# huiscliu/lssp

Hardware: AMD Instinct MI355X
Metric: fp64 CSR SpMV GB/s (% HBM peak) + BiCGSTAB iters/s, 7-pt Poisson n=10M (higher is better)
Workload: dtype f64; 1 GPU; 7-pt Poisson 216^3 (n=10077696, nnz=70263936), BiCGSTAB + ILUK(0), b=1, x0=0, fp64 CSR int32; rows=10077696, partition=1 z-slab row blocks, reduction=tree, transport=none, comm_ranks=1

## Files before the change

### include/lssp_amd.h

```cpp
#ifndef LSSP_AMD_H
#define LSSP_AMD_H

#ifdef __cplusplus
extern "C" {
#endif

enum {
    LSSP_AMD_OK = 0,
    LSSP_AMD_EINVAL = 1,
    LSSP_AMD_EHIP = 2,
    LSSP_AMD_ENOMEM = 3,
    LSSP_AMD_ETIMEOUT = 4,
    LSSP_AMD_ECOMM = 5,
    LSSP_AMD_EUNSUPPORTED = 6
};

enum {
    LSSP_AMD_REDUCE_SERIAL = 0,
    LSSP_AMD_REDUCE_TREE = 1
};

enum {
    LSSP_AMD_GMRES = 0, LSSP_AMD_LGMRES = 1, LSSP_AMD_RGMRES = 2, LSSP_AMD_RLGMRES = 3, LSSP_AMD_BICGSTAB = 4,
    LSSP_AMD_BICGSAFE = 6, LSSP_AMD_CG = 7, LSSP_AMD_CGS = 8, LSSP_AMD_GPBICG = 9, LSSP_AMD_CR = 10,
// ... 9 lines not shown

const char *lssp_amd_strerror(int status);
int lssp_amd_version(void);

void lssp_amd_set_print(int (*fn)(void *user, const char *msg), void *user);

int lssp_amd_ctx_create(int device, lssp_amd_ctx **ctx);
int lssp_amd_ctx_destroy(lssp_amd_ctx *ctx);
int lssp_amd_ctx_set_reduction(lssp_amd_ctx *ctx, int mode);
int lssp_amd_ctx_sync(lssp_amd_ctx *ctx);
void *lssp_amd_ctx_stream(lssp_amd_ctx *ctx);

int lssp_amd_vec_alloc(lssp_amd_ctx *ctx, long n, double **d);
int lssp_amd_vec_free(lssp_amd_ctx *ctx, double *d);
int lssp_amd_vec_upload(lssp_amd_ctx *ctx, double *d, const double *h, long n);
int lssp_amd_vec_download(lssp_amd_ctx *ctx, double *h, const double *d, long n);

int lssp_amd_csr_sort_columns(int nrows, int ncols, int *Ap, int *Aj, double *Ax);
int lssp_amd_mat_upload(lssp_amd_ctx *ctx, int nrows, int ncols, int nnz, const int *Ap,
                        const int *Aj, const double *Ax, lssp_amd_mat **A);
int lssp_amd_mat_destroy(lssp_amd_mat *A);
int lssp_amd_mat_info(const lssp_amd_mat *A, int *nrows, int *ncols, int *nnz);
int lssp_amd_mat_layout(const lssp_amd_mat *A, int *ndiag, int *windowed);
int lssp_amd_mat_bytes(const lssp_amd_mat *A, long long *csr_bytes, long long *aux_bytes);

int lssp_amd_mv_amxpby(lssp_amd_ctx *ctx, double alpha, const lssp_amd_mat *A, double *x,
                       double beta, double *y);
int lssp_amd_mv_amxpbyz(lssp_amd_ctx *ctx, double alpha, const lssp_amd_mat *A, double *x,
                        double beta, const double *y, double *z);
int lssp_amd_mv_amxy(lssp_amd_ctx *ctx, double a, const lssp_amd_mat *A, double *x, double *y);
int lssp_amd_mv_mxy(lssp_amd_ctx *ctx, const lssp_amd_mat *A, double *x, double *y);

int lssp_amd_vec_set_value(lssp_amd_ctx *ctx, double *x, long n, double val);
int lssp_amd_vec_copy(lssp_amd_ctx *ctx, double *x, const double *y, long n);
int lssp_amd_stream_read(lssp_amd_ctx *ctx, const double *x, long n, double *sink);
int lssp_amd_vec_axy(lssp_amd_ctx *ctx, double alpha, const double *x, double *y, long n);
int lssp_amd_vec_axpby(lssp_amd_ctx *ctx, double alpha, const double *x, double beta, double *y,
                       long n);
int lssp_amd_vec_axpbyz(lssp_amd_ctx *ctx, double alpha, const double *x, double beta,
                        const double *y, double *z, long n);
int lssp_amd_vec_scale(lssp_amd_ctx *ctx, double *x, long n, double a);
int lssp_amd_vec_dot(lssp_amd_ctx *ctx, const double *x, const double *y, long n, double *result);
int lssp_amd_vec_norm(lssp_amd_ctx *ctx, const double *x, long n, double *result);

int lssp_amd_ilu_create(lssp_amd_ctx *ctx, int kind, int n, const int *Ap, const int *Aj,
                        const double *Ax, int level, double tol, int p, int blk,
// ... 104 lines not shown
```

### lssp_amd/_lib.py

```python
from __future__ import annotations

import ctypes
import os

HERE = os.path.dirname(os.path.abspath(__file__))
LIB_PATH = os.environ.get("LSSP_AMD_LIB") or os.path.join(HERE, "lib", "liblssp_amd.so")
HEADER = os.path.join(os.path.dirname(HERE), "include", "lssp_amd.h")

_vp, _ci, _cd, _cl = ctypes.c_void_p, ctypes.c_int, ctypes.c_double, ctypes.c_long
_pvp = ctypes.POINTER(ctypes.c_void_p)


ALLGATHER_FN = ctypes.CFUNCTYPE(_ci, _vp, _vp, _vp, _cl)
SENDRECV_FN = ctypes.CFUNCTYPE(_ci, _vp, _ci, ctypes.POINTER(_ci), ctypes.POINTER(_vp), ctypes.POINTER(_cl),
                               _ci, ctypes.POINTER(_ci), ctypes.POINTER(_vp), ctypes.POINTER(_cl))


class HostTransport(ctypes.Structure):
    _fields_ = [("user", _vp), ("allgather", ALLGATHER_FN), ("sendrecv", SENDRECV_FN)]


class SolveParams(ctypes.Structure):
    _fields_ = [("solver", _ci), ("tol_rel", _cd), ("tol_abs", _cd), ("tol_rb", _cd),
                ("maxit", _ci), ("restart", _ci), ("verb", _ci), ("aug_k", _ci),
                ("bgsl", _ci), ("idrs", _ci)]


SIGNATURES = {
    "lssp_amd_strerror": (ctypes.c_char_p, [_ci]),
    "lssp_amd_version": (_ci, []),
    "lssp_amd_set_print": (None, [_vp, _vp]),
    "lssp_amd_ctx_create": (_ci, [_ci, _pvp]),
    "lssp_amd_ctx_destroy": (_ci, [_vp]),
    "lssp_amd_ctx_set_reduction": (_ci, [_vp, _ci]),
    "lssp_amd_ctx_sync": (_ci, [_vp]),
    "lssp_amd_ctx_stream": (_vp, [_vp]),
    "lssp_amd_vec_alloc": (_ci, [_vp, _cl, _pvp]),
    "lssp_amd_vec_free": (_ci, [_vp, _vp]),
    "lssp_amd_vec_upload": (_ci, [_vp, _vp, _vp, _cl]),
    "lssp_amd_vec_download": (_ci, [_vp, _vp, _vp, _cl]),
    "lssp_amd_csr_sort_columns": (_ci, [_ci, _ci, _vp, _vp, _vp]),
    "lssp_amd_mat_upload": (_ci, [_vp, _ci, _ci, _ci, _vp, _vp, _vp, _pvp]),
    "lssp_amd_mat_destroy": (_ci, [_vp]),
    "lssp_amd_mat_info": (_ci, [_vp, _vp, _vp, _vp]),
    "lssp_amd_mat_layout": (_ci, [_vp, _vp, _vp]),
    "lssp_amd_mat_bytes": (_ci, [_vp, _vp, _vp]),
    "lssp_amd_ilu_sweep_layout": (_ci, [_vp, _vp, _vp, _vp]),
    "lssp_amd_mv_amxpby": (_ci, [_vp, _cd, _vp, _vp, _cd, _vp]),
    "lssp_amd_mv_amxpbyz": (_ci, [_vp, _cd, _vp, _vp, _cd, _vp, _vp]),
    "lssp_amd_mv_amxy": (_ci, [_vp, _cd, _vp, _vp, _vp]),
    "lssp_amd_mv_mxy": (_ci, [_vp, _vp, _vp, _vp]),
    "lssp_amd_vec_set_value": (_ci, [_vp, _vp, _cl, _cd]),
    "lssp_amd_vec_copy": (_ci, [_vp, _vp, _vp, _cl]),
    "lssp_amd_stream_read": (_ci, [_vp, _vp, _cl, _vp]),
    "lssp_amd_vec_axy": (_ci, [_vp, _cd, _vp, _vp, _cl]),
    "lssp_amd_vec_axpby": (_ci, [_vp, _cd, _vp, _cd, _vp, _cl]),
    "lssp_amd_vec_axpbyz": (_ci, [_vp, _cd, _vp, _cd, _vp, _vp, _cl]),
    "lssp_amd_vec_scale": (_ci, [_vp, _vp, _cl, _cd]),
    "lssp_amd_vec_dot": (_ci, [_vp, _vp, _vp, _cl, _vp]),
    "lssp_amd_vec_norm": (_ci, [_vp, _vp, _cl, _vp]),
    "lssp_amd_ilu_create": (_ci, [_vp, _ci, _ci, _vp, _vp, _vp, _ci, _cd, _ci, _ci, _pvp]),
    "lssp_amd_ilu_from_factors": (_ci, [_vp, _ci, _vp, _vp, _vp, _vp, _vp, _vp, _pvp]),
    "lssp_amd_bilu_create": (_ci, [_vp, _ci, _vp, _vp, _vp, _ci, _ci, _pvp]),
    "lssp_amd_ilu_from_ldu": (_ci, [_vp, _ci, _vp, _vp, _vp, _vp, _vp, _vp, _vp, _vp, _vp, _pvp]),
    "lssp_amd_ilu_get_diag": (_ci, [_vp, _vp, _vp]),
    "lssp_amd_bilu_factor_host": (_ci, [_ci, _vp, _vp, _vp, _ci, _ci, _vp, _vp, _vp, _vp, _vp, _vp, _vp, _vp, _vp]),
    "lssp_amd_ilu_destroy": (_ci, [_vp]),
    "lssp_amd_ilu_apply": (_ci, [_vp, _vp, _vp, _vp]),
# ... 60 lines not shown
```

### lssp_amd/csrc/capi.cpp

```cpp
#include <hip/hip_runtime.h>

#include <algorithm>
#include <chrono>
#include <climits>
#include <cstdarg>
#include <atomic>
#include <cstdlib>
#include <cstring>
#include <exception>
#include <mutex>
#include <thread>

#include "bilu_dev.h"
#include "internal.h"

using namespace lssp_amd;

namespace lssp_amd {

long num_chunks(long n) { return (n + CHUNK - 1) / CHUNK; }

int ensure_part(lssp_amd_ctx *c, long C)
{
    if (C <= c->part_cap) return LSSP_AMD_OK;
// ... 406 lines not shown

static int check_csr(int nrows, int ncols, int nnz, const int *Ap, const int *Aj)
{
    if (nrows < 0 || ncols <= 0 || nnz < 0 || !Ap) return LSSP_AMD_EINVAL;
    if (Ap[0] != 0 || Ap[nrows] != nnz) return LSSP_AMD_EINVAL;
    for (int i = 0; i < nrows; i++)
        if (Ap[i + 1] < Ap[i]) return LSSP_AMD_EINVAL;
    for (int k = 0; k < nnz; k++)
        if (Aj[k] < 0 || Aj[k] >= ncols) return LSSP_AMD_EINVAL;
    return LSSP_AMD_OK;
}

static int upload_csr(lssp_amd_mat *M, const int *Ap, const int *Aj, const double *Ax)
{
    LSSP_HIP(hipMalloc(&M->Ap, sizeof(int) * (M->nrows + 1)));
    LSSP_HIP(hipMalloc(&M->Aj, sizeof(int) * (M->nnz + 4)));
    LSSP_HIP(hipMalloc(&M->Ax, sizeof(double) * (M->nnz + 4)));
    LSSP_HIP(hipMemcpy(M->Ap, Ap, sizeof(int) * (M->nrows + 1), hipMemcpyHostToDevice));
    if (M->nnz) {
        LSSP_HIP(hipMemcpy(M->Aj, Aj, sizeof(int) * M->nnz, hipMemcpyHostToDevice));
        LSSP_HIP(hipMemcpy(M->Ax, Ax, sizeof(double) * M->nnz, hipMemcpyHostToDevice));
    }
    LSSP_TRY(build_diag_ids(M, Ap, Aj));
    return build_windows(M, Ap, Aj, Ax);
}

int lssp_amd_mat_upload(lssp_amd_ctx *c, int nrows, int ncols, int nnz, const int *Ap, const int *Aj,
                        const double *Ax, lssp_amd_mat **out)
{
    if (!c || !out) return LSSP_AMD_EINVAL;
    LSSP_TRY(check_csr(nrows, ncols, nnz, Ap, Aj));
    LSSP_HIP(hipSetDevice(c->device));
    lssp_amd_mat *M = new lssp_amd_mat();
    M->ctx = c;
    M->nrows = nrows;
    M->ncols = ncols;
    M->nnz = nnz;
    M->n_global = nrows;
    int st = upload_csr(M, Ap, Aj, Ax);
    if (st != LSSP_AMD_OK) {
        lssp_amd_mat_destroy(M);
        return st;
    }
    if (tune_spmv_streams(c, M) != LSSP_AMD_OK) (void)hipGetLastError();
    *out = M;
    return LSSP_AMD_OK;
}

int lssp_amd_mat_destroy(lssp_amd_mat *M)
{
    if (!M) return LSSP_AMD_OK;
    if (M->ctx) (void)hipStreamSynchronize(M->ctx->stream);
    if (M->Ap) (void)hipFree(M->Ap);
    if (M->Aj) (void)hipFree(M->Aj);
    if (M->Ax) (void)hipFree(M->Ax);
    if (M->Ad) (void)hipFree(M->Ad);
    if (M->d_off) (void)hipFree(M->d_off);
    if (M->d_win) (void)hipFree(M->d_win);
    for (void *p : {(void *)M->s_ax, (void *)M->s_col, (void *)M->s_row, (void *)M->s_meta})
        if (p) (void)hipFree(p);
    if (M->d_send_idx) (void)hipFree(M->d_send_idx);
    if (M->d_send_buf) (void)hipFree(M->d_send_buf);
    delete M;
    return LSSP_AMD_OK;
}

int lssp_amd_mat_info(const lssp_amd_mat *A, int *nrows, int *ncols, int *nnz)
{
    if (!A) return LSSP_AMD_EINVAL;
    if (nrows) *nrows = A->nrows;
    if (ncols) *ncols = A->ncols;
    if (nnz) *nnz = A->nnz;
    return LSSP_AMD_OK;
}

int lssp_amd_mat_bytes(const lssp_amd_mat *A, long long *csr_bytes, long long *aux_bytes)
{
    if (!A) return LSSP_AMD_EINVAL;
    if (csr_bytes) *csr_bytes = 4LL * (A->nrows + 1) + 12LL * A->nnz;
    if (aux_bytes) *aux_bytes = A->aux_bytes;
    return LSSP_AMD_OK;
}

int lssp_amd_mat_layout(const lssp_amd_mat *A, int *ndiag, int *windowed)
{
    if (!A || !ndiag) return LSSP_AMD_EINVAL;
    *ndiag = A->ndiag;
    if (windowed) *windowed = A->d_win != nullptr;
    return LSSP_AMD_OK;
}

int lssp_amd_mat_local_rows(const lssp_amd_mat *A, int *row0, int *nlocal, int *nhalo)
{
    if (!A) return LSSP_AMD_EINVAL;
    if (row0) *row0 = A->row0;
    if (nlocal) *nlocal = A->nrows;
    if (nhalo) *nhalo = A->nhalo;
    return LSSP_AMD_OK;
}

int lssp_amd_mv_amxpby(lssp_amd_ctx *c, double alpha, const lssp_amd_mat *A, double *x,
                       double beta, double *y)
{
    if (!c || !A || !x || !y) return LSSP_AMD_EINVAL;
    return spmv_halo(c, A, EPI_AXPBY, alpha, x, beta, y, y, 0, nullptr, nullptr);
}

int lssp_amd_mv_amxpbyz(lssp_amd_ctx *c, double alpha, const lssp_amd_mat *A, double *x,
                        double beta, const double *y, double *z)
{
    if (!c || !A || !x || !y || !z) return LSSP_AMD_EINVAL;
// ... 755 lines not shown
```

### lssp_amd/csrc/comm.cpp

```cpp
#include <hip/hip_runtime.h>
#include <rccl/rccl.h>

#include <algorithm>
#include <climits>
#include <cstring>
#include <map>

#include "internal.h"

namespace lssp_amd {

#define LSSP_NCCL(call)                                                                            \
    do {                                                                                           \
        ncclResult_t r_ = (call);                                                                  \
        if (r_ != ncclSuccess) {                                                                   \
            fprintf(stderr, "lssp_amd: RCCL error %s at %s:%d\n", ncclGetErrorString(r_), __FILE__, \
                    __LINE__);                                                                     \
            return LSSP_AMD_ECOMM;                                                                 \
        }                                                                                          \
    } while (0)

struct Msg {
    int peer;
    void *dbuf;
// ... 458 lines not shown
    if (nsend)
        LSSP_HIP(hipMemcpyAsync(sendg.data(), d_sendg.p, sizeof(int) * nsend, hipMemcpyDeviceToHost, c->stream));
    LSSP_HIP(hipStreamSynchronize(c->stream));
    st = LSSP_AMD_OK;
    for (int &g : sendg) {
        if (g < row0 || g >= row0 + nlocal) st = LSSP_AMD_EINVAL;
        g -= row0;
    }
    LSSP_TRY(agree_status(c, st));
    auto dev_ok = [](hipError_t e) { return e == hipSuccess; };
    const bool ok =
        dev_ok(hipMalloc(&M->d_send_idx, sizeof(int) * std::max(nsend, 1))) &&
        dev_ok(hipMalloc(&M->d_send_buf, sizeof(double) * std::max(nsend, 1))) &&
        (!nsend || dev_ok(hipMemcpy(M->d_send_idx, sendg.data(), sizeof(int) * nsend, hipMemcpyHostToDevice))) &&
        dev_ok(hipMalloc(&M->Ap, sizeof(int) * (nlocal + 1))) &&
        dev_ok(hipMalloc(&M->Aj, sizeof(int) * ((size_t)nnz + 4))) &&
        dev_ok(hipMalloc(&M->Ax, sizeof(double) * ((size_t)nnz + 4))) &&
        dev_ok(hipMemcpy(M->Ap, Ap, sizeof(int) * (nlocal + 1), hipMemcpyHostToDevice)) &&
        (!nnz || (dev_ok(hipMemcpy(M->Aj, lj.data(), sizeof(int) * (size_t)nnz, hipMemcpyHostToDevice)) &&
                  dev_ok(hipMemcpy(M->Ax, Ax, sizeof(double) * (size_t)nnz, hipMemcpyHostToDevice))));
    if (!ok) (void)hipGetLastError();
    LSSP_TRY(agree_status(c, ok ? LSSP_AMD_OK : LSSP_AMD_ENOMEM));
    LSSP_TRY(agree_status(c, build_diag_ids(M, Ap, lj.data())));
    guard.m = nullptr;
    *out = M;
    return LSSP_AMD_OK;
}

}
```

### lssp_amd/csrc/convert.hip

```cpp
#include <hip/hip_runtime.h>
#include <rocprim/device/device_radix_sort.hpp>
#include <rocprim/device/device_scan.hpp>

#include <algorithm>
#include <cstdint>
#include <cstdlib>
#include <vector>

#include "internal.h"

namespace {

constexpr int CT = 256;

unsigned grid_for(long n)
{
    long b = (n + CT - 1) / CT;
    return (unsigned)std::max<long>(1, std::min<long>(b, 16384));
}

#define GRID_STRIDE(i, n) for (long i = blockIdx.x * (long)CT + threadIdx.x; i < (n); i += (long)gridDim.x * CT)

int bits_for(unsigned long v)
{
// ... 443 lines not shown
__global__ __launch_bounds__(CT) void k_off_ids(long nrows, const int *__restrict__ Ap, const int *__restrict__ Aj,
                                                const int *__restrict__ off, int nd, uint8_t *__restrict__ Ad)
{
    __shared__ int tab[DIAG_MAX + 1];
    for (int t = threadIdx.x; t < nd; t += CT) tab[t] = off[t];
    __syncthreads();
    GRID_STRIDE(i, nrows)
    {
        int e = Ap[i + 1];
        for (int k = Ap[i]; k < e; k++) {
            int o = Aj[k] - (int)i, lo = 0, hi = nd - 1;
            while (lo < hi) {
                int mid = (lo + hi) >> 1;
                if (tab[mid] < o)
                    lo = mid + 1;
                else
                    hi = mid;
            }
            Ad[k] = (uint8_t)lo;
        }
    }
}

__global__ __launch_bounds__(CT) void k_win_wide(long nb, int nrows, const int *__restrict__ Ap,
                                                 const int *__restrict__ Aj, int *__restrict__ wide)
{
    __shared__ int slo, shi;
    for (long b = blockIdx.x; b < nb; b += gridDim.x) {
        if (threadIdx.x == 0) slo = INT32_MAX, shi = INT32_MIN;
        __syncthreads();
        long r0 = b * lssp_amd::WIN_ROWS, r1 = r0 + lssp_amd::WIN_ROWS < nrows ? r0 + lssp_amd::WIN_ROWS : nrows;
        int lo = INT32_MAX, hi = INT32_MIN;
        for (int k = Ap[r0] + threadIdx.x; k < Ap[r1]; k += CT) {
            lo = min(lo, Aj[k]);
            hi = max(hi, Aj[k]);
        }
        if (lo <= hi) {
            atomicMin(&slo, lo);
            atomicMax(&shi, hi);
        }
        __syncthreads();
        if (threadIdx.x == 0 && slo <= shi && (long)shi + 1 - (slo & ~1) > lssp_amd::WIN_CAP) atomicOr(wide, 1);
        __syncthreads();
    }
}

// ... 84 lines not shown
}

#define TRY(x)                     \
    do {                           \
        int st_ = (x);             \
        if (st_) return st_;       \
    } while (0)

int bucket(Scratch &S, long nnz, const int *key, int nr, const int *sj, const double *sx, int *P, int *dj,
           double *dx)
{
    hipStream_t s = S.s;
    SCRATCH(idx, int, nnz);
    SCRATCH(perm, int, nnz);
    SCRATCH(skey, unsigned, nnz);
    k_iota<<<grid_for(nnz), CT, 0, s>>>(nnz, idx);
    TRY(sort_pairs(S, (const unsigned *)key, skey, (const int *)idx, perm, nnz, bits_for((unsigned)std::max(nr - 1, 0))));
    k_row_ptr<<<grid_for((long)nr + 1), CT, 0, s>>>(nr, skey, (int)nnz, P);
    k_gather<<<grid_for(nnz), CT, 0, s>>>(nnz, perm, sj, sx, dj, dx);
    LSSP_HIP(hipGetLastError());
    return LSSP_AMD_OK;
}

}

extern "C" {

int lssp_amd_idx_alloc(lssp_amd_ctx *c, long n, int **d)
{
    if (!c || !d || n < 0) return LSSP_AMD_EINVAL;
    if (hipMalloc(d, sizeof(int) * std::max<long>(n, 1)) != hipSuccess) return LSSP_AMD_ENOMEM;
    return LSSP_AMD_OK;
}

int lssp_amd_idx_free(lssp_amd_ctx *c, int *d)
{
    if (!c) return LSSP_AMD_EINVAL;
    LSSP_HIP(hipStreamSynchronize(c->stream));
    if (d) LSSP_HIP(hipFree(d));
    return LSSP_AMD_OK;
}

int lssp_amd_idx_upload(lssp_amd_ctx *c, int *d, const int *h, long n)
{
    if (!c || n < 0 || (n > 0 && (!d || !h))) return LSSP_AMD_EINVAL;
    if (n == 0) return LSSP_AMD_OK;
// ... 302 lines not shown
    SCRATCH(g, int, G_SIZE);
    k_off_init<<<1, CT, 0, s>>>(g);
    k_off_collect<<<grid_for(M->nrows), CT, 0, s>>>(M->nrows, M->Ap, M->Aj, g);
    LSSP_HIP(hipGetLastError());
    int head[2 + DIAG_MAX];
    LSSP_HIP(hipMemcpyAsync(head, g + G_COUNT, sizeof(head), hipMemcpyDeviceToHost, s));
    LSSP_HIP(hipStreamSynchronize(s));
    if (head[1] || head[0] > DIAG_MAX) return LSSP_AMD_OK;
    std::vector<int> off(head + 2, head + 2 + head[0]);
    std::sort(off.begin(), off.end());
    const size_t ad_bytes = (size_t)M->nnz + 32;
    LSSP_HIP(hipMalloc(&M->Ad, ad_bytes));
    LSSP_HIP(hipMalloc(&M->d_off, sizeof(int) * off.size()));
    LSSP_HIP(hipMemsetAsync(M->Ad + M->nnz, 0, 32, s));
    LSSP_HIP(hipMemcpyAsync(M->d_off, off.data(), sizeof(int) * off.size(), hipMemcpyHostToDevice, s));
    k_off_ids<<<grid_for(M->nrows), CT, 0, s>>>(M->nrows, M->Ap, M->Aj, M->d_off, (int)off.size(), M->Ad);
    LSSP_HIP(hipGetLastError());
    LSSP_HIP(hipStreamSynchronize(s));
    M->aux_bytes += (long long)ad_bytes + (long long)sizeof(int) * (long long)off.size();
    M->ndiag = (int)off.size();
    M->max_off = 0;
    for (int o : off) M->max_off = std::max(M->max_off, std::abs(o));
    M->max_off_int = M->max_off;
    return LSSP_AMD_OK;
}

static int windows_dev(lssp_amd_ctx *c, lssp_amd_mat *M)
{
    if (M->ndiag > 0 || M->nnz == 0 || M->nrows == 0) return LSSP_AMD_OK;
    hipStream_t s = c->stream;
    {
        Scratch S(s);
        SCRATCH(wide, int, 1);
        LSSP_HIP(hipMemsetAsync(wide, 0, sizeof(int), s));
        const long nb = ((long)M->nrows + lssp_amd::WIN_ROWS - 1) / lssp_amd::WIN_ROWS;
        k_win_wide<<<(unsigned)std::min<long>(nb, 16384), CT, 0, s>>>(nb, M->nrows, M->Ap, M->Aj, wide);
        LSSP_HIP(hipGetLastError());
        int h = 0;
        TRY(fetch(s, wide, &h));
        if (h) return LSSP_AMD_OK;
    }
    std::vector<int> Ap((size_t)M->nrows + 1), Aj((size_t)M->nnz);
    std::vector<double> Ax((size_t)M->nnz);
    LSSP_HIP(hipMemcpyAsync(Ap.data(), M->Ap, sizeof(int) * Ap.size(), hipMemcpyDeviceToHost, s));
    LSSP_HIP(hipMemcpyAsync(Aj.data(), M->Aj, sizeof(int) * Aj.size(), hipMemcpyDeviceToHost, s));
    LSSP_HIP(hipMemcpyAsync(Ax.data(), M->Ax, sizeof(double) * Ax.size(), hipMemcpyDeviceToHost, s));
    LSSP_HIP(hipStreamSynchronize(s));
// ... 68 lines not shown
```

### lssp_amd/csrc/internal.h

```cpp
#pragma once

#include <hip/hip_runtime.h>

#include <cstdint>
#include <cstdio>
#include <functional>
#include <mutex>
#include <string>
#include <vector>

#include "../../include/lssp_amd.h"

namespace lssp_amd {

constexpr int CHUNK = 256;
constexpr int L2_LANES = 1024;
constexpr int MAX_SLOTS = 4;
constexpr int NSCAL = 4096;

constexpr uint64_t TRI_SENTINEL = 0xFFF7DEADBEEFCAFEull;

enum Scal {
    S_RHO0 = 0, S_RHO1, S_ALPHA, S_BETA, S_OMEGA, S_RES, S_SNORM, S_BREAK, S_BNORM, S_TMP,
    S_DONE, S_TOL, S_NIT,
// ... 53 lines not shown
    double *d_gather = nullptr;
    double *d_carry = nullptr;
    int *d_igather = nullptr;
    hipStream_t comm_stream = nullptr;
    hipEvent_t ev_pack = nullptr, ev_halo = nullptr;
    int tri_blocks_per_cu = 1;
    struct WsBuf {
        double *p;
        long n;
        bool used;
    };
    std::vector<WsBuf> pool;
};

struct lssp_amd_mat {
    lssp_amd_ctx *ctx = nullptr;
    int nrows = 0, ncols = 0, nnz = 0;
    int *Ap = nullptr, *Aj = nullptr;
    double *Ax = nullptr;
    uint8_t *Ad = nullptr;
    int *d_off = nullptr;
    int ndiag = 0;
    int max_off = 0;
    int max_off_int = 0;
    int *d_win = nullptr;
    double *s_ax = nullptr;
    uint32_t *s_col = nullptr, *s_row = nullptr;
    int *s_meta = nullptr;
    long long aux_bytes = 0;
    int streams = 0;
    int n_global = 0, row0 = 0, nhalo = 0;
    bool dist = false;
    std::vector<int> send_peer, send_off, send_cnt;
    std::vector<int> recv_peer, recv_off, recv_cnt;
    int *d_send_idx = nullptr;
    double *d_send_buf = nullptr;
    int nsend = 0;
    long ich0 = 0, ich1 = 0;
};

namespace lssp_amd {

struct TriSched {
    int n = 0, nnz = 0, nlevels = 0, unit = 0, upper = 0;
    int *perm = nullptr;
    int *rp = nullptr;
// ... 120 lines not shown

#define LSSP_HIP(call)                                                                    \
    do {                                                                                  \
        hipError_t e_ = (call);                                                           \
        if (e_ != hipSuccess) {                                                           \
            fprintf(stderr, "lssp_amd: HIP error %s at %s:%d\n", hipGetErrorString(e_), \
                    __FILE__, __LINE__);                                                  \
            return LSSP_AMD_EHIP;                                                         \
        }                                                                                 \
    } while (0)

#define LSSP_TRY(call)               \
    do {                             \
        int s_ = (call);             \
        if (s_ != LSSP_AMD_OK) return s_; \
    } while (0)

enum Epi { EPI_MXY = 0, EPI_AMXY, EPI_AXPBY, EPI_AMX };
int build_diag_ids(lssp_amd_mat *M, const int *Ap, const int *Aj);
int build_windows(lssp_amd_mat *M, const int *Ap, const int *Aj, const double *Ax);
int tune_spmv_streams(lssp_amd_ctx *c, lssp_amd_mat *M);
constexpr int WIN_ROWS = 1024, WIN_CAP = 16384;
constexpr int DIAG_MAX = 255, DIAG_HS = 1024;
int launch_spmv(lssp_amd_ctx *c, const lssp_amd_mat *A, int epi, double alpha, const double *x,
                double beta, const double *y, double *z, int nred, const double *w0,
                const double *w1, long cb = 0, long ce = -1);
struct Ew {
    int kind = 0;
    long n = 0;
    double a = 0, b = 0;
    const double *x = nullptr, *y = nullptr, *u = nullptr, *v = nullptr;
    double *out0 = nullptr, *out1 = nullptr;
    const double *scal = nullptr;
    int nred = 0;
    const double *r0a = nullptr, *r0b = nullptr, *r1a = nullptr, *r1b = nullptr;
    const double *r2a = nullptr, *r2b = nullptr, *r3a = nullptr, *r3b = nullptr;
    const double *vbase = nullptr;
    int k = 0;
    int sidx = 0;
    int pslot = 0;
};
int launch_ew(lssp_amd_ctx *c, const Ew &e);
int launch_copy(lssp_amd_ctx *c, double *x, const double *y, long n);
int launch_stream_read(lssp_amd_ctx *c, const double *x, long n, double *sink);

int launch_reduce_tree(lssp_amd_ctx *c, long C, int nslot, const Fin &f, int slot0 = 0);
// ... 177 lines not shown
```

### lssp_amd/csrc/kernels.hip

```cpp
#include <hip/hip_runtime.h>

#include <algorithm>
#include <climits>
#include <vector>

#include <cstdint>
#include <cstring>
#include <string>
#include <type_traits>

#include "internal.h"

namespace lssp_amd {

__device__ __forceinline__ double wave_sum(double v)
{
    return wave_sum_l0(v);
}

template <int NRED>
__device__ __forceinline__ void chunk_reduce(double (&v)[NRED > 0 ? NRED : 1], double *part, long pcap,
                                             long chunk, double (*lds)[4])
{
    const int lane = threadIdx.x & 63, wave = threadIdx.x >> 6;
// ... 257 lines not shown
    }
    finalize(f, r, scal, trace);
}

constexpr int SPMV_CAP = 2048;

struct SpmvArgs {
    int nrows;
    const int *Ap, *Aj;
    const double *Ax, *x, *y;
    double *z;
    double alpha, beta;
    const double *w0, *w1;
    double *part;
    long pcap;
    const uint8_t *Ad;
    const int *off;
    int ndiag;
    const double *guard;
    long blk0;
    int streams;
    int pbpp, pz, pw;
    int ntv;
};

template <int EPI, int NRED, bool CMP>
__global__ __launch_bounds__(256) void k_spmv3(SpmvArgs a, long nblk, long nnz_pad)
{
    constexpr int NX2 = (SPMV_CAP / 2 + 1 + 255) / 256;
    constexpr int NJ4 = CMP ? 1 : (SPMV_CAP / 4 + 1 + 255) / 256;
    __shared__ __attribute__((aligned(16))) double sx[SPMV_CAP + 2];
    __shared__ __attribute__((aligned(16))) int sj[CMP ? SPMV_CAP / 4 + 8 : SPMV_CAP + 4];
    __shared__ int soff[CMP ? 256 : 1];
    __shared__ double lds[MAX_SLOTS][4];
    const double gv = a.guard ? *a.guard : 0.0;
    const long per = gridDim.x / a.streams;
    long lb = (blockIdx.x % a.streams) * per + blockIdx.x / a.streams;
    if (lb >= nblk) return;
    if (a.pbpp > 0 && lb < (long)a.pbpp * a.pz) {
        const long gs = (long)a.pw * a.pz, g = lb / gs, rem = lb - g * gs;
        lb = (rem / a.pw) * a.pbpp + g * a.pw + rem % a.pw;
    }
    const long blk = a.blk0 + lb;
    const int r0 = (int)(blk * 256);
    const int tid = threadIdx.x;
    const int r = r0 + tid;
    const int rend = min(r0 + 256, a.nrows);
    const int base = a.Ap[r0];
    const int cnt = a.Ap[rend] - base;
    const int rr = min(r, a.nrows - 1);
    const int rb = a.Ap[rr], re = a.Ap[rr + 1];
    double w0p = 0.0, w1p = 0.0;
    if (NRED > 0) {
        if (a.ntv) {
            if (a.w0 != a.z) w0p = __builtin_nontemporal_load(a.w0 + rr);
            if (NRED > 1 && a.w1 && a.w1 != a.z) w1p = __builtin_nontemporal_load(a.w1 + rr);
        } else {
            if (a.w0 != a.z) w0p = a.w0[rr];
            if (NRED > 1 && a.w1 && a.w1 != a.z) w1p = a.w1[rr];
        }
    }
    if (gv != 0.0) return;
    double sum = 0;
    if (cnt <= SPMV_CAP) {
        typedef double dbl2_t __attribute__((ext_vector_type(2)));
        typedef int int4_t __attribute__((ext_vector_type(4)));
        constexpr int JS = CMP ? 4 : 2;
        const long xb = base & ~1L, jb = base & ~((1L << JS) - 1);
        const long last = cnt > 0 ? (long)base + cnt - 1 : (long)base;
        const long xmax = min(last >> 1, (nnz_pad >> 1) - 1);
        const long jmax = min(last >> JS, (CMP ? (nnz_pad - 4 + 32) >> 4 : nnz_pad >> 2) - 1);
        if (CMP && tid < a.ndiag) soff[tid] = a.off[tid];
        const dbl2_t *X2 = reinterpret_cast<const dbl2_t *>(a.Ax);
        const int4_t *J4 = CMP ? reinterpret_cast<const int4_t *>(a.Ad) : reinterpret_cast<const int4_t *>(a.Aj);
        dbl2_t vx[NX2];
        int4_t vj[NJ4];
#pragma unroll
        for (int u = 0; u < NX2; u++) vx[u] = __builtin_nontemporal_load(X2 + min((xb >> 1) + tid + 256 * u, xmax));
#pragma unroll
        for (int u = 0; u < NJ4; u++) vj[u] = __builtin_nontemporal_load(J4 + min((jb >> JS) + tid + 256 * u, jmax));
        const int xn = (int)(xmax - (xb >> 1)) + 1, jn = (int)(jmax - (jb >> JS)) + 1;
#pragma unroll
        for (int u = 0; u < NX2; u++)
            if (tid + 256 * u < xn) reinterpret_cast<dbl2_t *>(sx)[tid + 256 * u] = vx[u];
#pragma unroll
        for (int u = 0; u < NJ4; u++)
            if (tid + 256 * u < jn) reinterpret_cast<int4_t *>(sj)[tid + 256 * u] = vj[u];
        __syncthreads();
        if (r < a.nrows) {
            const int ox = (int)(base - xb) - base, oj = (int)(base - jb) - base;
            const int len = re - rb;
            const unsigned char *sd = reinterpret_cast<const unsigned char *>(sj);
            auto col = [&](int k) { return CMP ? r + soff[sd[k + oj]] : sj[k + oj]; };
            if (len > 0 && len <= 8) {
                double pr[8];
#pragma unroll
                for (int u = 0; u < 8; u++) {
                    const int k = min(rb + u, re - 1);
                    pr[u] = a.x[col(k)] * sx[k + ox];
                }
#pragma unroll
                for (int u = 0; u < 8; u++)
                    if (u < len) sum += pr[u];
            } else {
                for (int k = rb; k < re; k++) sum += a.x[col(k)] * sx[k + ox];
            }
        }
    } else if (r < a.nrows) {
        for (int k = rb; k < re; k++) sum += a.x[a.Aj[k]] * a.Ax[k];
    }
    double zv = 0;
    if (r < a.nrows) {
// ... 179 lines not shown
        return e ? std::max(0, atoi(e)) : -1;
    }();
    return k;
}

static int spmv_ntv()
{
    static const int k = [] {
        const char *e = getenv("LSSP_AMD_SPMV_NTV");
        return e ? atoi(e) : 1;
    }();
    return k;
}

static int spmv_streams_env()
{
    static const int k = [] {
        const char *e = getenv("LSSP_AMD_SPMV_STREAMS");
        const int v = e ? atoi(e) : 0;
        return v >= 8 && v % 8 == 0 && v <= 4096 ? v : 0;
    }();
    return k;
}
static int spmv_streams(const lssp_amd_mat *A)
{
    const int e = spmv_streams_env();
    return e ? e : A->streams > 0 ? A->streams : 8;
}

template <int EPI, bool CMP>
static void spmv_dispatch(const SpmvArgs &a, int nred, long nblocks, hipStream_t s, long nnz_pad)
{
    const long g = (nblocks + a.streams - 1) / a.streams * a.streams;
    if (nred == 0) k_spmv3<EPI, 0, CMP><<<g, 256, 0, s>>>(a, nblocks, nnz_pad);
    else if (nred == 1) k_spmv3<EPI, 1, CMP><<<g, 256, 0, s>>>(a, nblocks, nnz_pad);
    else if (nred == 2 || EPI != EPI_AMX) k_spmv3<EPI, 2, CMP><<<g, 256, 0, s>>>(a, nblocks, nnz_pad);
    else k_spmv3<EPI_AMX, 3, CMP><<<g, 256, 0, s>>>(a, nblocks, nnz_pad);
}

template <int EPI>
static void spmv_dispatch(const SpmvArgs &a, int nred, long nblocks, hipStream_t s, long nnz_pad)
{
    if (a.ndiag > 0) spmv_dispatch<EPI, true>(a, nred, nblocks, s, nnz_pad);
    else spmv_dispatch<EPI, false>(a, nred, nblocks, s, nnz_pad);
}

int launch_spmv(lssp_amd_ctx *c, const lssp_amd_mat *A, int epi, double alpha, const double *x,
                double beta, const double *y, double *z, int nred, const double *w0,
                const double *w1, long cb, long ce)
{
    if (A->nrows == 0) return LSSP_AMD_OK;
    const long nall = num_chunks(A->nrows);
    LSSP_TRY(ensure_part(c, nall));
    if (ce < 0) ce = nall;
    if (cb < 0 || cb > ce || ce > nall) return LSSP_AMD_EINVAL;
    if (nred == 3 && (epi != EPI_AMX || !w0 || w0 == z || w1)) return LSSP_AMD_EINVAL;
    const long nb = ce - cb;
    if (nb == 0) return LSSP_AMD_OK;
    SpmvArgs a{A->nrows, A->Ap, A->Aj, A->Ax, x, y, z, alpha, beta, w0, w1, c->d_part, c->part_cap,
               A->Ad, A->d_off, A->ndiag, c->guard, cb, spmv_streams(A), 0, 0, 0, spmv_ntv()};
    const long plane = A->max_off_int;
    if (A->ndiag > 0 && plane >= 256 * 8 && plane % 256 == 0) {
        const long bpp = plane / 256;
        const int env = spmv_group_env();
        const int pw = env >= 0 ? env : (bpp >= 512 && bpp % 128 == 0 ? 128 : 0);
        if (pw > 0 && bpp % pw == 0 && nb / bpp >= 2) {
            a.pbpp = (int)bpp;
            a.pz = (int)(nb / bpp);
            a.pw = pw;
        }
    }
    if (A->d_win && nb == nall && nred <= 2) {
        switch (epi) {
        case EPI_MXY: spmv_sell_dispatch<EPI_MXY>(a, A, nred, c->stream, c->num_cus); break;
        case EPI_AMXY: spmv_sell_dispatch<EPI_AMXY>(a, A, nred, c->stream, c->num_cus); break;
        case EPI_AXPBY: spmv_sell_dispatch<EPI_AXPBY>(a, A, nred, c->stream, c->num_cus); break;
        default: spmv_sell_dispatch<EPI_AMX>(a, A, nred, c->stream, c->num_cus); break;
        }
        LSSP_HIP(hipGetLastError());
        return LSSP_AMD_OK;
    }
    switch (epi) {
    case EPI_MXY: spmv_dispatch<EPI_MXY>(a, nred, nb, c->stream, A->nnz + 4L); break;
// ... 536 lines not shown
```

### lssp_amd/device.py

```python
from __future__ import annotations

import ctypes
import weakref
from dataclasses import dataclass

import numpy as np

from . import _lib

GMRES, LGMRES, RGMRES, BICGSTAB, CG = 0, 1, 2, 4, 7
BICGSAFE, CGS, GPBICG, CR, CRS, BICRSTAB, BICRSAFE, GPBICR, QMRCGSTAB, TFQMR, ORTHOMIN = (
    6, 8, 9, 10, 11, 12, 13, 14, 15, 16, 17)
BICGSTABL, IDRS = 5, 18
RLGMRES = 3
ILUK, ILUT, BILUK = 1, 2, 3
SERIAL, TREE = 0, 1


class LsspError(RuntimeError):
    def __init__(self, status: int, what: str):
        msg = _lib.load().lssp_amd_strerror(status).decode()
        super().__init__(f"{what}: {msg} (status {status})")
        self.status = status

# ... 178 lines not shown
        dev._adopt(self)
        r0, nl, nh = ctypes.c_int(), ctypes.c_int(), ctypes.c_int()
        dev.L.lssp_amd_mat_local_rows(h, ctypes.byref(r0), ctypes.byref(nl), ctypes.byref(nh))
        self.row0, self.nrows, self.nhalo = r0.value, nl.value, nh.value
        self.nnz = nnz

    @classmethod
    def from_device(cls, dev: Device, nrows: int, ncols: int, nnz: int, Ap: "DIdx", Aj: "DIdx", Ax: "DVec"):
        h = ctypes.c_void_p()
        _ck(dev.L.lssp_amd_mat_from_device(dev.h, nrows, ncols, nnz, Ap.ptr, Aj.ptr, Ax.ptr, ctypes.byref(h)),
            "mat_from_device")
        self = cls.__new__(cls)
        self._adopt_handle(dev, h, int(nnz))
        return self

    @property
    def nx(self) -> int:
        return self.nrows + self.nhalo

    @property
    def ndiag(self) -> int:
        v, w = ctypes.c_int(), ctypes.c_int()
        _ck(self.dev.L.lssp_amd_mat_layout(self.h, ctypes.byref(v), ctypes.byref(w)), "mat_layout")
        return v.value

    @property
    def windowed(self) -> bool:
        v, w = ctypes.c_int(), ctypes.c_int()
        _ck(self.dev.L.lssp_amd_mat_layout(self.h, ctypes.byref(v), ctypes.byref(w)), "mat_layout")
        return bool(w.value)

    @property
    def device_bytes(self) -> tuple[int, int]:
        c, a = ctypes.c_longlong(), ctypes.c_longlong()
        _ck(self.dev.L.lssp_amd_mat_bytes(self.h, ctypes.byref(c), ctypes.byref(a)), "mat_bytes")
        return c.value, a.value

    def update_values(self, ax: DVec):
        _ck(self.dev.L.lssp_amd_mat_update_values(self.dev.h, self.h, ax.ptr, ax.n), "mat_update_values")

    def close(self):
        if self.h:
            self.dev.L.lssp_amd_mat_destroy(self.h)
            self.h = None

    def __del__(self):
# ... 178 lines not shown
```

Measured before the change: 680.0 iters/s.

## Encode per-row diagonal patterns as one-byte codes to shrink SpMV index traffic

```diff
diff --git a/include/lssp_amd.h b/include/lssp_amd.h
--- a/include/lssp_amd.h
+++ b/include/lssp_amd.h
@@ -55,6 +55,7 @@
 int lssp_amd_mat_destroy(lssp_amd_mat *A);
 int lssp_amd_mat_info(const lssp_amd_mat *A, int *nrows, int *ncols, int *nnz);
 int lssp_amd_mat_layout(const lssp_amd_mat *A, int *ndiag, int *windowed);
+int lssp_amd_mat_rowcodes(const lssp_amd_mat *A, int *npatterns);
 int lssp_amd_mat_bytes(const lssp_amd_mat *A, long long *csr_bytes, long long *aux_bytes);
 
 int lssp_amd_mv_amxpby(lssp_amd_ctx *ctx, double alpha, const lssp_amd_mat *A, double *x,
diff --git a/lssp_amd/_lib.py b/lssp_amd/_lib.py
--- a/lssp_amd/_lib.py
+++ b/lssp_amd/_lib.py
@@ -44,6 +44,7 @@
     "lssp_amd_mat_destroy": (_ci, [_vp]),
     "lssp_amd_mat_info": (_ci, [_vp, _vp, _vp, _vp]),
     "lssp_amd_mat_layout": (_ci, [_vp, _vp, _vp]),
+    "lssp_amd_mat_rowcodes": (_ci, [_vp, _vp]),
     "lssp_amd_mat_bytes": (_ci, [_vp, _vp, _vp]),
     "lssp_amd_ilu_sweep_layout": (_ci, [_vp, _vp, _vp, _vp]),
     "lssp_amd_mv_amxpby": (_ci, [_vp, _cd, _vp, _vp, _cd, _vp]),
diff --git a/lssp_amd/csrc/capi.cpp b/lssp_amd/csrc/capi.cpp
--- a/lssp_amd/csrc/capi.cpp
+++ b/lssp_amd/csrc/capi.cpp
@@ -452,6 +452,7 @@
         LSSP_HIP(hipMemcpy(M->Ax, Ax, sizeof(double) * M->nnz, hipMemcpyHostToDevice));
     }
     LSSP_TRY(build_diag_ids(M, Ap, Aj));
+    LSSP_TRY(build_row_codes(M->ctx, M));
     return build_windows(M, Ap, Aj, Ax);
 }
 
@@ -486,6 +487,8 @@
     if (M->Ax) (void)hipFree(M->Ax);
     if (M->Ad) (void)hipFree(M->Ad);
     if (M->d_off) (void)hipFree(M->d_off);
+    if (M->Ac) (void)hipFree(M->Ac);
+    if (M->d_pat) (void)hipFree(M->d_pat);
     if (M->d_win) (void)hipFree(M->d_win);
     for (void *p : {(void *)M->s_ax, (void *)M->s_col, (void *)M->s_row, (void *)M->s_meta})
         if (p) (void)hipFree(p);
@@ -517,6 +520,13 @@
     if (!A || !ndiag) return LSSP_AMD_EINVAL;
     *ndiag = A->ndiag;
     if (windowed) *windowed = A->d_win != nullptr;
+    return LSSP_AMD_OK;
+}
+
+int lssp_amd_mat_rowcodes(const lssp_amd_mat *A, int *npatterns)
+{
+    if (!A || !npatterns) return LSSP_AMD_EINVAL;
+    *npatterns = A->npat;
     return LSSP_AMD_OK;
 }
 
diff --git a/lssp_amd/csrc/comm.cpp b/lssp_amd/csrc/comm.cpp
--- a/lssp_amd/csrc/comm.cpp
+++ b/lssp_amd/csrc/comm.cpp
@@ -504,6 +504,7 @@
     if (!ok) (void)hipGetLastError();
     LSSP_TRY(agree_status(c, ok ? LSSP_AMD_OK : LSSP_AMD_ENOMEM));
     LSSP_TRY(agree_status(c, build_diag_ids(M, Ap, lj.data())));
+    LSSP_TRY(agree_status(c, build_row_codes(c, M)));
     guard.m = nullptr;
     *out = M;
     return LSSP_AMD_OK;
diff --git a/lssp_amd/csrc/convert.hip b/lssp_amd/csrc/convert.hip
--- a/lssp_amd/csrc/convert.hip
+++ b/lssp_amd/csrc/convert.hip
@@ -489,6 +489,101 @@
     }
 }
 
+using lssp_amd::ROWPAT_LEN;
+using lssp_amd::ROWPAT_MAX;
+typedef unsigned long long pat_t;
+constexpr pat_t PAT_EMPTY = ~0ull;
+constexpr int PAT_HS = 1024;
+constexpr int P_COUNT = 0, P_OVER = 1;
+
+__device__ __forceinline__ unsigned pat_slot(pat_t k) { return (unsigned)((k * 0x9E3779B97F4A7C15ull) >> 54); }
+
+__global__ __launch_bounds__(CT) void k_pat_init(pat_t *__restrict__ gk, int *__restrict__ gi)
+{
+    for (int t = threadIdx.x; t < PAT_HS + ROWPAT_MAX; t += CT) gk[t] = t < PAT_HS ? PAT_EMPTY : 0;
+    if (threadIdx.x < 2) gi[threadIdx.x] = 0;
+}
+
+__device__ __forceinline__ bool pat_insert(pat_t *tab, const int *full, pat_t k)
+{
+    unsigned h = pat_slot(k);
+    for (int p = 0; p < PAT_HS; p++, h = (h + 1) & (PAT_HS - 1)) {
+        pat_t cur = *(volatile pat_t *)(tab + h);
+        if (cur == k) return false;
+        if (cur != PAT_EMPTY) continue;
+        if (*(volatile const int *)full > ROWPAT_MAX) return false;
+        pat_t old = atomicCAS(tab + h, PAT_EMPTY, k);
+        if (old == PAT_EMPTY) return true;
+        if (old == k) return false;
+    }
+    return false;
+}
+
+__device__ __forceinline__ pat_t pat_key(const uint8_t *__restrict__ Ad, int b, int e)
+{
+    pat_t key = 0;
+    for (int k = b; k < e; k++) key |= (pat_t)(Ad[k] + 1u) << (8 * (k - b));
+    return key;
+}
+
+__global__ __launch_bounds__(CT) void k_pat_collect(long nrows, const int *__restrict__ Ap,
+                                                    const uint8_t *__restrict__ Ad, pat_t *__restrict__ gk,
+                                                    int *__restrict__ gi)
+{
+    __shared__ pat_t tab[PAT_HS];
+    __shared__ int cnt;
+    for (int t = threadIdx.x; t < PAT_HS; t += CT) tab[t] = PAT_EMPTY;
+    if (threadIdx.x == 0) cnt = 0;
+    __syncthreads();
+    GRID_STRIDE(i, nrows)
+    {
+        if (*(volatile int *)&cnt > ROWPAT_MAX || *(volatile int *)(gi + P_OVER)) break;
+        const int b = Ap[i], e = Ap[i + 1];
+        const pat_t key = e - b <= ROWPAT_LEN ? pat_key(Ad, b, e) : PAT_EMPTY;
+        if (key == PAT_EMPTY) {
+            atomicOr(gi + P_OVER, 1);
+            break;
+        }
+        if (pat_insert(tab, &cnt, key)) atomicAdd(&cnt, 1);
+    }
+    __syncthreads();
+    if (cnt > ROWPAT_MAX) {
+        if (threadIdx.x == 0) atomicOr(gi + P_OVER, 1);
+        return;
+    }
+    for (int t = threadIdx.x; t < PAT_HS; t += CT) {
+        pat_t k = tab[t];
+        if (k == PAT_EMPTY || !pat_insert(gk, gi + P_COUNT, k)) continue;
+        int at = atomicAdd(gi + P_COUNT, 1);
+        if (at < ROWPAT_MAX)
+            gk[PAT_HS + at] = k;
+        else
+            atomicOr(gi + P_OVER, 1);
+    }
+}
+
+__global__ __launch_bounds__(CT) void k_pat_codes(long nrows, const int *__restrict__ Ap,
+                                                  const uint8_t *__restrict__ Ad, const pat_t *__restrict__ pat,
+                                                  int np, uint8_t *__restrict__ Ac)
+{
+    __shared__ pat_t tab[ROWPAT_MAX];
+    for (int t = threadIdx.x; t < np; t += CT) tab[t] = pat[t];
+    __syncthreads();
+    GRID_STRIDE(i, nrows)
+    {
+        const pat_t key = pat_key(Ad, Ap[i], Ap[i + 1]);
+        int lo = 0, hi = np - 1;
+        while (lo < hi) {
+            int mid = (lo + hi) >> 1;
+            if (tab[mid] < key)
+                lo = mid + 1;
+            else
+                hi = mid;
+        }
+        Ac[i] = (uint8_t)lo;
+    }
+}
+
 __global__ __launch_bounds__(CT) void k_win_wide(long nb, int nrows, const int *__restrict__ Ap,
                                                  const int *__restrict__ Aj, int *__restrict__ wide)
 {
@@ -619,6 +714,43 @@
     return LSSP_AMD_OK;
 }
 
+}
+
+int lssp_amd::build_row_codes(lssp_amd_ctx *c, lssp_amd_mat *M)
+{
+    M->npat = 0;
+    if (M->ndiag == 0 || !M->Ad || M->nnz == 0 || M->nrows == 0) return LSSP_AMD_OK;
+    hipStream_t s = c->stream;
+    Scratch S(s);
+    SCRATCH(gk, pat_t, PAT_HS + ROWPAT_MAX);
+    SCRATCH(gi, int, 2);
+    k_pat_init<<<1, CT, 0, s>>>(gk, gi);
+    k_pat_collect<<<grid_for(M->nrows), CT, 0, s>>>(M->nrows, M->Ap, M->Ad, gk, gi);
+    LSSP_HIP(hipGetLastError());
+    int head[2];
+    std::vector<pat_t> pat(ROWPAT_MAX);
+    LSSP_HIP(hipMemcpyAsync(head, gi, sizeof(head), hipMemcpyDeviceToHost, s));
+    LSSP_HIP(hipMemcpyAsync(pat.data(), gk + PAT_HS, sizeof(pat_t) * ROWPAT_MAX, hipMemcpyDeviceToHost, s));
+    LSSP_HIP(hipStreamSynchronize(s));
+    if (head[P_OVER] || head[P_COUNT] > ROWPAT_MAX || head[P_COUNT] <= 0) return LSSP_AMD_OK;
+    pat.resize(head[P_COUNT]);
+    std::sort(pat.begin(), pat.end());
+    const size_t ac_bytes = (size_t)M->nrows + 32;
+    LSSP_HIP(hipMalloc(&M->Ac, ac_bytes));
+    LSSP_HIP(hipMalloc(&M->d_pat, sizeof(pat_t) * pat.size()));
+    LSSP_HIP(hipMemsetAsync(M->Ac + M->nrows, 0, 32, s));
+    LSSP_HIP(hipMemcpyAsync(M->d_pat, pat.data(), sizeof(pat_t) * pat.size(), hipMemcpyHostToDevice, s));
+    k_pat_codes<<<grid_for(M->nrows), CT, 0, s>>>(M->nrows, M->Ap, M->Ad, M->d_pat, (int)pat.size(), M->Ac);
+    LSSP_HIP(hipGetLastError());
+    LSSP_HIP(hipStreamSynchronize(s));
+    for (int l = 0; l < ROWPAT_LEN; l++) {
+        int shorter = 0;
+        for (pat_t k : pat) shorter += (k >> (8 * l)) == 0;
+        M->pat_thr[l] = (unsigned short)shorter;
+    }
+    M->aux_bytes += (long long)ac_bytes + (long long)sizeof(pat_t) * (long long)pat.size();
+    M->npat = (int)pat.size();
+    return LSSP_AMD_OK;
 }
 
 extern "C" {
@@ -967,7 +1099,7 @@
     M->max_off = 0;
     for (int o : off) M->max_off = std::max(M->max_off, std::abs(o));
     M->max_off_int = M->max_off;
-    return LSSP_AMD_OK;
+    return lssp_amd::build_row_codes(c, M);
 }
 
 static int windows_dev(lssp_amd_ctx *c, lssp_amd_mat *M)
diff --git a/lssp_amd/csrc/internal.h b/lssp_amd/csrc/internal.h
--- a/lssp_amd/csrc/internal.h
+++ b/lssp_amd/csrc/internal.h
@@ -99,6 +99,10 @@
     int *d_off = nullptr;
     int ndiag = 0;
     int max_off = 0;
+    uint8_t *Ac = nullptr;
+    unsigned long long *d_pat = nullptr;
+    int npat = 0;
+    unsigned short pat_thr[8] = {0, 0, 0, 0, 0, 0, 0, 0};
     int max_off_int = 0;
     int *d_win = nullptr;
     double *s_ax = nullptr;
@@ -265,6 +269,8 @@
 int tune_spmv_streams(lssp_amd_ctx *c, lssp_amd_mat *M);
 constexpr int WIN_ROWS = 1024, WIN_CAP = 16384;
 constexpr int DIAG_MAX = 255, DIAG_HS = 1024;
+constexpr int ROWPAT_MAX = 256, ROWPAT_LEN = 8;
+int build_row_codes(lssp_amd_ctx *c, lssp_amd_mat *M);
 int launch_spmv(lssp_amd_ctx *c, const lssp_amd_mat *A, int epi, double alpha, const double *x,
                 double beta, const double *y, double *z, int nred, const double *w0,
                 const double *w1, long cb = 0, long ce = -1);
diff --git a/lssp_amd/csrc/kernels.hip b/lssp_amd/csrc/kernels.hip
--- a/lssp_amd/csrc/kernels.hip
+++ b/lssp_amd/csrc/kernels.hip
@@ -303,16 +303,25 @@
     int streams;
     int pbpp, pz, pw;
     int ntv;
+    const uint8_t *Ac;
+    const unsigned long long *pat;
+    int npat;
+    unsigned short thr[8];
 };
 
-template <int EPI, int NRED, bool CMP>
+enum { COL_J = 0, COL_ID = 1, COL_ROW = 2 };
+template <int EPI, int NRED, int CM>
 __global__ __launch_bounds__(256) void k_spmv3(SpmvArgs a, long nblk, long nnz_pad)
 {
+    constexpr bool CMP = CM == COL_ID, ROW = CM == COL_ROW;
+    static_assert(256 * 8 <= SPMV_CAP, "a row-coded block fits the staging buffer");
     constexpr int NX2 = (SPMV_CAP / 2 + 1 + 255) / 256;
     constexpr int NJ4 = CMP ? 1 : (SPMV_CAP / 4 + 1 + 255) / 256;
     __shared__ __attribute__((aligned(16))) double sx[SPMV_CAP + 2];
-    __shared__ __attribute__((aligned(16))) int sj[CMP ? SPMV_CAP / 4 + 8 : SPMV_CAP + 4];
-    __shared__ int soff[CMP ? 256 : 1];
+    __shared__ __attribute__((aligned(16))) int sj[ROW ? 1 : CMP ? SPMV_CAP / 4 + 8 : SPMV_CAP + 4];
+    __shared__ int soff[CM != COL_J ? 256 : 1];
+    __shared__ unsigned long long spat[ROW ? 256 : 1];
+    __shared__ int swt[ROW ? 4 : 1];
     __shared__ double lds[MAX_SLOTS][4];
     const double gv = a.guard ? *a.guard : 0.0;
     const long per = gridDim.x / a.streams;
@@ -330,7 +339,10 @@
     const int base = a.Ap[r0];
     const int cnt = a.Ap[rend] - base;
     const int rr = min(r, a.nrows - 1);
-    const int rb = a.Ap[rr], re = a.Ap[rr + 1];
+    int rb = 0, re = 0;
+    unsigned code = 0;
+    if (ROW) code = a.Ac[rr];
+    else rb = a.Ap[rr], re = a.Ap[rr + 1];
     double w0p = 0.0, w1p = 0.0;
     if (NRED > 0) {
         if (a.ntv) {
@@ -343,7 +355,7 @@
     }
     if (gv != 0.0) return;
     double sum = 0;
-    if (cnt <= SPMV_CAP) {
+    if (ROW || cnt <= SPMV_CAP) {
         typedef double dbl2_t __attribute__((ext_vector_type(2)));
         typedef int int4_t __attribute__((ext_vector_type(4)));
         constexpr int JS = CMP ? 4 : 2;
@@ -351,24 +363,62 @@
         const long last = cnt > 0 ? (long)base + cnt - 1 : (long)base;
         const long xmax = min(last >> 1, (nnz_pad >> 1) - 1);
         const long jmax = min(last >> JS, (CMP ? (nnz_pad - 4 + 32) >> 4 : nnz_pad >> 2) - 1);
-        if (CMP && tid < a.ndiag) soff[tid] = a.off[tid];
+        if (CM != COL_J && tid < a.ndiag) soff[tid] = a.off[tid];
+        if (ROW && tid < a.npat) spat[tid] = a.pat[tid];
         const dbl2_t *X2 = reinterpret_cast<const dbl2_t *>(a.Ax);
         const int4_t *J4 = CMP ? reinterpret_cast<const int4_t *>(a.Ad) : reinterpret_cast<const int4_t *>(a.Aj);
         dbl2_t vx[NX2];
-        int4_t vj[NJ4];
+        int4_t vj[ROW ? 1 : NJ4];
 #pragma unroll
         for (int u = 0; u < NX2; u++) vx[u] = __builtin_nontemporal_load(X2 + min((xb >> 1) + tid + 256 * u, xmax));
-#pragma unroll
-        for (int u = 0; u < NJ4; u++) vj[u] = __builtin_nontemporal_load(J4 + min((jb >> JS) + tid + 256 * u, jmax));
+        if (!ROW) {
+#pragma unroll
+            for (int u = 0; u < NJ4; u++) vj[u] = __builtin_nontemporal_load(J4 + min((jb >> JS) + tid + 256 * u, jmax));
+        }
         const int xn = (int)(xmax - (xb >> 1)) + 1, jn = (int)(jmax - (jb >> JS)) + 1;
+        int len = 0, inc = 0;
+        if (ROW) {
+#pragma unroll
+            for (int l = 0; l < 8; l++) len += code >= (unsigned)a.thr[l];
+            if (r >= a.nrows) len = 0;
+            const int lane = tid & 63;
+            inc = len;
+#pragma unroll
+            for (int d = 1; d < 64; d <<= 1) {
+                const int t = __shfl_up(inc, d, 64);
+                if (lane >= d) inc += t;
+            }
+            if (lane == 63) swt[tid >> 6] = inc;
+        }
 #pragma unroll
         for (int u = 0; u < NX2; u++)
             if (tid + 256 * u < xn) reinterpret_cast<dbl2_t *>(sx)[tid + 256 * u] = vx[u];
-#pragma unroll
-        for (int u = 0; u < NJ4; u++)
-            if (tid + 256 * u < jn) reinterpret_cast<int4_t *>(sj)[tid + 256 * u] = vj[u];
+        if (!ROW) {
+#pragma unroll
+            for (int u = 0; u < NJ4; u++)
+                if (tid + 256 * u < jn) reinterpret_cast<int4_t *>(sj)[tid + 256 * u] = vj[u];
+        }
         __syncthreads();
-        if (r < a.nrows) {
+        if (ROW) {
+            if (len > 0) {
+                const int wave = tid >> 6;
+                int lo = inc - len;
+                if (wave > 0) lo += swt[0];
+                if (wave > 1) lo += swt[1];
+                if (wave > 2) lo += swt[2];
+                const double *sr = sx + ((int)(base - xb) + lo);
+                const unsigned long long pt = spat[code];
+                double pr[8];
+#pragma unroll
+                for (int u = 0; u < 8; u++) {
+                    const int k = min(u, len - 1);
+                    pr[u] = a.x[r + soff[(int)((pt >> (8 * k)) & 255u) - 1]] * sr[k];
+                }
+#pragma unroll
+                for (int u = 0; u < 8; u++)
+                    if (u < len) sum += pr[u];
+            }
+        } else if (r < a.nrows) {
             const int ox = (int)(base - xb) - base, oj = (int)(base - jb) - base;
             const int len = re - rb;
             const unsigned char *sd = reinterpret_cast<const unsigned char *>(sj);
@@ -594,27 +644,36 @@
     }();
     return k;
 }
+static int spmv_rowcode()
+{
+    static const int k = [] {
+        const char *e = getenv("LSSP_AMD_SPMV_ROWCODE");
+        return e ? atoi(e) : 1;
+    }();
+    return k;
+}
 static int spmv_streams(const lssp_amd_mat *A)
 {
     const int e = spmv_streams_env();
     return e ? e : A->streams > 0 ? A->streams : 8;
 }
 
-template <int EPI, bool CMP>
+template <int EPI, int CM>
 static void spmv_dispatch(const SpmvArgs &a, int nred, long nblocks, hipStream_t s, long nnz_pad)
 {
     const long g = (nblocks + a.streams - 1) / a.streams * a.streams;
-    if (nred == 0) k_spmv3<EPI, 0, CMP><<<g, 256, 0, s>>>(a, nblocks, nnz_pad);
-    else if (nred == 1) k_spmv3<EPI, 1, CMP><<<g, 256, 0, s>>>(a, nblocks, nnz_pad);
-    else if (nred == 2 || EPI != EPI_AMX) k_spmv3<EPI, 2, CMP><<<g, 256, 0, s>>>(a, nblocks, nnz_pad);
-    else k_spmv3<EPI_AMX, 3, CMP><<<g, 256, 0, s>>>(a, nblocks, nnz_pad);
+    if (nred == 0) k_spmv3<EPI, 0, CM><<<g, 256, 0, s>>>(a, nblocks, nnz_pad);
+    else if (nred == 1) k_spmv3<EPI, 1, CM><<<g, 256, 0, s>>>(a, nblocks, nnz_pad);
+    else if (nred == 2 || EPI != EPI_AMX) k_spmv3<EPI, 2, CM><<<g, 256, 0, s>>>(a, nblocks, nnz_pad);
+    else k_spmv3<EPI_AMX, 3, CM><<<g, 256, 0, s>>>(a, nblocks, nnz_pad);
 }
 
 template <int EPI>
 static void spmv_dispatch(const SpmvArgs &a, int nred, long nblocks, hipStream_t s, long nnz_pad)
 {
-    if (a.ndiag > 0) spmv_dispatch<EPI, true>(a, nred, nblocks, s, nnz_pad);
-    else spmv_dispatch<EPI, false>(a, nred, nblocks, s, nnz_pad);
+    if (a.npat > 0) spmv_dispatch<EPI, COL_ROW>(a, nred, nblocks, s, nnz_pad);
+    else if (a.ndiag > 0) spmv_dispatch<EPI, COL_ID>(a, nred, nblocks, s, nnz_pad);
+    else spmv_dispatch<EPI, COL_J>(a, nred, nblocks, s, nnz_pad);
 }
 
 int launch_spmv(lssp_amd_ctx *c, const lssp_amd_mat *A, int epi, double alpha, const double *x,
@@ -630,7 +689,14 @@
     const long nb = ce - cb;
     if (nb == 0) return LSSP_AMD_OK;
     SpmvArgs a{A->nrows, A->Ap, A->Aj, A->Ax, x, y, z, alpha, beta, w0, w1, c->d_part, c->part_cap,
-               A->Ad, A->d_off, A->ndiag, c->guard, cb, spmv_streams(A), 0, 0, 0, spmv_ntv()};
+               A->Ad, A->d_off, A->ndiag, c->guard, cb, spmv_streams(A), 0, 0, 0, spmv_ntv(),
+               nullptr, nullptr, 0, {0, 0, 0, 0, 0, 0, 0, 0}};
+    if (A->npat > 0 && spmv_rowcode()) {
+        a.Ac = A->Ac;
+        a.pat = A->d_pat;
+        a.npat = A->npat;
+        memcpy(a.thr, A->pat_thr, sizeof(a.thr));
+    }
     const long plane = A->max_off_int;
     if (A->ndiag > 0 && plane >= 256 * 8 && plane % 256 == 0) {
         const long bpp = plane / 256;
diff --git a/lssp_amd/device.py b/lssp_amd/device.py
--- a/lssp_amd/device.py
+++ b/lssp_amd/device.py
@@ -224,6 +224,12 @@
     def ndiag(self) -> int:
         v, w = ctypes.c_int(), ctypes.c_int()
         _ck(self.dev.L.lssp_amd_mat_layout(self.h, ctypes.byref(v), ctypes.byref(w)), "mat_layout")
+        return v.value
+
+    @property
+    def rowcodes(self) -> int:
+        v = ctypes.c_int()
+        _ck(self.dev.L.lssp_amd_mat_rowcodes(self.h, ctypes.byref(v)), "mat_rowcodes")
         return v.value
 
     @property
```

Result: faster. 697.0 iters/s (median of 6 runs) (+2.5%).
